# autonomousvision/connecting_the_dots

Measured on AMD Instinct MI355X. Metric: Mpix*disparities/s on 512x432x128 cost volume; disparity MAE vs ref, higher is better.
Workload: dtype f32

## Files before the change

### connecting_the_dots_amd/csrc/argmax_rerank.hip

```cpp
#include "ctd_internal.h"
#include "ctd_ncc_point.h"
#include "ctd_rank.h"
#include "ctd_tail.h"


namespace ctd {

constexpr int kScanBatch = 8;
template <int PX>
__global__ __launch_bounds__(256) __attribute__((amdgpu_waves_per_eu(5, 8))) void argmax_scan_kernel(const float* __restrict__ vol, int64_t* __restrict__ idx,
                                                          float* __restrict__ best, int D, long HW, int W,
                                                          int bs, float eps, long total_threads, WorkList work) {
  const long t = (long)blockIdx.x * blockDim.x + threadIdx.x;
  if (t >= total_threads) return;
  const long p0 = t * PX;
  const long f = p0 / HW, q0 = p0 - f * HW;
  const float* v = vol + f * D * HW + q0;
  const int w0 = (int)(q0 % W);
  float v0[PX], v1[PX];
  int i0[PX], dc[PX];
#pragma unroll
  for (int k = 0; k < PX; ++k) { v0[k] = -INFINITY; v1[k] = -INFINITY; i0[k] = 0; dc[k] = w0 + k + (bs - 1 - bs / 2); }
  constexpr int kBatch = kScanBatch;
  const bool wave_masks = __any(dc[0] < D - 1);
  for (int d0 = 0; d0 < D; d0 += kBatch) {
    float x[kBatch][PX];
#pragma unroll
    for (int u = 0; u < kBatch; ++u) {
      const float* src = v + (long)min(d0 + u, D - 1) * HW;
      if constexpr (PX == 4) {
        typedef float f4 __attribute__((ext_vector_type(4)));
        const f4 q = __builtin_nontemporal_load((const f4*)src);
        x[u][0] = q.x; x[u][1] = q.y; x[u][2] = q.z; x[u][3] = q.w;
      } else if constexpr (PX == 2) {
        typedef float f2 __attribute__((ext_vector_type(2)));
        const f2 q = __builtin_nontemporal_load((const f2*)src);
        x[u][0] = q.x; x[u][1] = q.y;
      } else {
        x[u][0] = __builtin_nontemporal_load(src);
      }
    }
    if (wave_masks || d0 + kBatch > D) {
#pragma unroll
      for (int u = 0; u < kBatch; ++u) {
        const int d = d0 + u;
#pragma unroll
        for (int k = 0; k < PX; ++k) {
          const float y = (d > dc[k] || d >= D) ? -INFINITY : x[u][k];
          v1[k] = __builtin_amdgcn_fmed3f(v0[k], v1[k], y);
          i0[k] = y > v0[k] ? d : i0[k];
          v0[k] = fmaxf(v0[k], y);
        }
      }
    } else {
#pragma unroll
      for (int u = 0; u < kBatch; ++u) {
#pragma unroll
        for (int k = 0; k < PX; ++k) {
          const float y = x[u][k];
          v1[k] = __builtin_amdgcn_fmed3f(v0[k], v1[k], y);
          i0[k] = y > v0[k] ? d0 + u : i0[k];
          v0[k] = fmaxf(v0[k], y);
        }
      }
    }
  }
#pragma unroll
  for (int k = 0; k < PX; ++k) {
    const bool hard = v1[k] >= v0[k] - eps;
    idx[p0 + k] = hard ? (int64_t)(-1 - i0[k]) : (int64_t)i0[k];
    if (best) best[p0 + k] = v0[k];
    if (hard) work.list[atomicAdd(work.counters, 1u)] = p0 + k;
  }
}

constexpr int kMaskWords = 8;

__device__ inline float wave_maxf(float v) {
#pragma unroll
  for (int o = 32; o > 0; o >>= 1) v = fmaxf(v, __shfl_xor(v, o));
  return v;
}

struct RunSource {
  const float* run_vals;
  const float* v1;
  int W1, xoff, per_frame;
};

template <int WORDS, bool VOL>
__device__ __forceinline__ void resolve_role(float* lds_resolve, const float* __restrict__ vol, const float* __restrict__ in0,
                                             const float* __restrict__ in1, long in1_frame_stride,
                                             int64_t* __restrict__ idx, float* __restrict__ best, int D, int H, int W, int bs,
                                             float eps, WorkList work, RunSource rsrc, unsigned role_block,
                                             unsigned n_role_blocks, unsigned waves_used = 4, unsigned* stamp = nullptr) {
  if ((threadIdx.x >> 6) >= waves_used) return;
  const int lane = threadIdx.x & 63;
  const int half = bs / 2, span = bs + D - 1;
  float* sA = lds_resolve + (threadIdx.x >> 6) * 2 * (bs * bs + bs * span);
  float* sB = sA + bs * bs;
  float* sAq = sB + bs * span;
  float* sBq = sAq + bs * bs;
  const float bs2f = (float)(bs * bs);
  const long HW = (long)H * W;
  unsigned seg_cnt[kWorkListParts];
  unsigned longest = 0;
#pragma unroll
  for (int k = 0; k < kWorkListParts; ++k) seg_cnt[k] = work.counters[min(k, work.parts - 1) * kWorkListStride];
#pragma unroll
  for (int k = 0; k < kWorkListParts; ++k) {
    if (k >= work.parts) seg_cnt[k] = 0u;
    longest = max(longest, seg_cnt[k]);
  }
  const unsigned n_slots = longest * (unsigned)work.parts;
  CTD_POST_STAMP_S(stamp, 1, longest);
  const unsigned n_waves = n_role_blocks * waves_used;
  for (unsigned slot = role_block * waves_used + (threadIdx.x >> 6); slot < n_slots; slot += n_waves) {
    const unsigned seg = slot & (unsigned)(work.parts - 1), entry = slot / (unsigned)work.parts;
    unsigned cnt = 0;
#pragma unroll
    for (int k = 0; k < kWorkListParts; ++k) cnt = seg == (unsigned)k ? seg_cnt[k] : cnt;
    if (entry >= cnt) continue;
    const long pj = work.list[(long)seg * work.seg_cap + entry];
    CTD_POST_STAMP_S(stamp, 2, pj);
    CTD_POST_STAMP_ITEM(stamp);
    const long fj = pj / HW, qj = pj - fj * HW;
    const int hj = (int)(qj / W), wj = (int)(qj - (long)hj * W);
    const float* v = VOL ? vol + fj * D * HW + qj : nullptr;
    const int d_clamped = wj + (bs - 1 - bs / 2);
    unsigned long long mask[WORDS];
    int n_cand = 0;
    float x[WORDS];
    bool run_listed = false;
    float rv = 0.f;
    if constexpr (VOL) {
      if (rsrc.run_vals && d_clamped < D) {
        const long z = rsrc.per_frame ? fj : 0;
        run_listed = rsrc.v1[(z * H + hj) * rsrc.W1 + (rsrc.xoff - (bs - 1 - bs / 2))] == 0.f;
        if (run_listed) rv = rsrc.run_vals[(fj * H + hj) * D + d_clamped];
      }
#pragma unroll
      for (int wd = 0; wd < WORDS; ++wd) {
        const int d = min(wd * 64 + lane, D - 1);
        x[wd] = v[(long)(rsrc.run_vals ? min(d, d_clamped) : d) * HW];
        if (run_listed && d >= d_clamped) x[wd] = rv;
      }
      CTD_POST_STAMP_V(stamp, 3, x[0]);
    }
    constexpr int kPreA = 2, kPreB = 20;
    const bool pre = !VOL && bs * bs <= 64 * kPreA && bs * span <= 64 * kPreB;
    const float* a = in0 + fj * HW;
    const float* b = in1 + fj * in1_frame_stride;
    float ta[kPreA], tb[kPreB];
    if (pre) {
#pragma unroll
      for (int k = 0; k < kPreA; ++k) {
        const int i = min(lane + 64 * k, bs * bs - 1);
        const int bh = i / bs, bw = i - bh * bs;
        ta[k] = a[(long)clampi(hj + bh - half, 0, H - 1) * W + clampi(wj + bw - half, 0, W - 1)];
      }
#pragma unroll
      for (int k = 0; k < kPreB; ++k) {
        const int i = min(lane + 64 * k, bs * span - 1);
        const int bh = i / span, c = i - bh * span;
        tb[k] = b[(long)clampi(hj + bh - half, 0, H - 1) * W + clampi(wj - half - (D - 1) + c, 0, W - 1)];
      }
    }
    if constexpr (VOL) {
      float m = -INFINITY;
#pragma unroll
      for (int wd = 0; wd < WORDS; ++wd)
        if (wd * 64 + lane < D && wd * 64 + lane <= d_clamped) m = fmaxf(m, x[wd]);
      m = wave_maxf(m);
      bool have_clamped = false;
#pragma unroll
      for (int wd = 0; wd < WORDS; ++wd) {
        unsigned long long bits = __ballot(wd * 64 + lane < D && x[wd] >= m - eps);
        const int c0 = d_clamped - wd * 64;
        if (c0 < 64) {
          const unsigned long long run = c0 <= 0 ? bits : bits & ~((1ull << c0) - 1ull);
          bits &= ~run;
          if (!have_clamped && run) {
            bits |= run & (0ull - run);
            have_clamped = true;
          }
        }
        mask[wd] = bits;
        n_cand += __popcll(bits);
      }
    } else {
#pragma unroll
      for (int wd = 0; wd < WORDS; ++wd) {
        const int last = min(D - 1, d_clamped) - wd * 64;
        mask[wd] = last < 0 ? 0ull : (last >= 63 ? ~0ull : ((1ull << (last + 1)) - 1ull));
        n_cand += __popcll(mask[wd]);
      }
    }
    float eb = 0.f;
    int ei = 0x7fffffff;
    const bool rescore = VOL ? n_cand > 1 : n_cand >= 1;
    if (rescore && pre) {
#pragma unroll
      for (int k = 0; k < kPreA; ++k)
        if (lane + 64 * k < bs * bs) {
          sA[lane + 64 * k] = ta[k];
          sAq[lane + 64 * k] = ta[k] / bs2f;
        }
#pragma unroll
      for (int k = 0; k < kPreB; ++k)
        if (lane + 64 * k < bs * span) {
          sB[lane + 64 * k] = tb[k];
          sBq[lane + 64 * k] = tb[k] / bs2f;
        }
    } else if (rescore) {
      for (int i = lane; i < bs * bs; i += 64) {
        const int bh = i / bs, bw = i - bh * bs;
        const float xa = a[(long)clampi(hj + bh - half, 0, H - 1) * W + clampi(wj + bw - half, 0, W - 1)];
        sA[i] = xa;
        sAq[i] = xa / bs2f;
      }
      constexpr int NB = 20;
      for (int i0 = lane; i0 < bs * span; i0 += 64 * NB) {
        float t[NB];
#pragma unroll
        for (int k = 0; k < NB; ++k) {
          const int i = min(i0 + 64 * k, bs * span - 1);
          const int bh = i / span, c = i - bh * span;
          t[k] = b[(long)clampi(hj + bh - half, 0, H - 1) * W + clampi(wj - half - (D - 1) + c, 0, W - 1)];
        }
#pragma unroll
        for (int k = 0; k < NB; ++k)
          if (i0 + 64 * k < bs * span) {
            sB[i0 + 64 * k] = t[k];
            sBq[i0 + 64 * k] = t[k] / bs2f;
          }
      }
    }
    CTD_POST_STAMP(stamp, 4);
    if (rescore) {
      for (int c0 = 0; c0 < n_cand; c0 += 64) {
        int my_d = -1, k = 0;
#pragma unroll
        for (int wd = 0; wd < WORDS; ++wd) {
          unsigned long long mj = mask[wd];
          if (k + __popcll(mj) <= c0 || k >= c0 + 64) { k += __popcll(mj); continue; }
          while (mj) {
            const int d = wd * 64 + __ffsll((long long)mj) - 1;
            mj &= mj - 1;
            if (k - c0 == lane) my_d = d;
            ++k;
          }
        }
        float e = -INFINITY;
        if (my_d >= 0) e = bs == 9 ? ncc_exact_point_lds_bs<9>(sA, sB, sAq, sBq, span, (D - 1) - my_d)
                                   : ncc_exact_point_lds(sA, sB, bs, span, (D - 1) - my_d);
        const float em = wave_maxf(e);
        const unsigned long long holders = __ballot(my_d >= 0 && e == em);
        const int dl = __shfl(my_d, holders ? __ffsll((long long)holders) - 1 : 0);
        if (ei == 0x7fffffff || em > eb) { eb = em; ei = dl; }
      }
    } else {
#pragma unroll
      for (int wd = 0; wd < WORDS; ++wd)
        if (mask[wd]) ei = min(ei, wd * 64 + __ffsll((long long)mask[wd]) - 1);
    }
    CTD_POST_STAMP_S(stamp, 5, ei);
    if (lane == 0) {
      idx[pj] = ei;
      if (best) {
        if constexpr (VOL) best[pj] = (run_listed && ei >= d_clamped) ? rv : v[(long)(rsrc.run_vals ? min(ei, d_clamped) : ei) * HW];
        else if (rescore) best[pj] = eb;
      }
    }
    CTD_POST_STAMP(stamp, 6);
    CTD_POST_STAMP(stamp, 9);
    stamp = nullptr;
  }
}

template <int WORDS, bool VOL>
__global__ __launch_bounds__(256) void argmax_resolve_kernel(const float* __restrict__ vol, const float* __restrict__ in0,
                                                             const float* __restrict__ in1, long in1_frame_stride,
                                                             int64_t* __restrict__ idx, float* __restrict__ best, int D,
                                                             int H, int W, int bs, float eps, WorkList work) {
  extern __shared__ float lds_dyn[];
  resolve_role<WORDS, VOL>(lds_dyn, vol, in0, in1, in1_frame_stride, idx, best, D, H, W, bs, eps, work,
                           RunSource{nullptr, nullptr, 0, 0, 0}, blockIdx.x, gridDim.x);
}

constexpr long kResolveBlocks = 1024;
constexpr unsigned kTailResolveWaves = 2;

template <int WORDS, bool VOL>
__global__ __launch_bounds__(256) void rank_tail_kernel(float* __restrict__ vol, const float* __restrict__ in0,
                                                        const float* __restrict__ in1, long in1_frame_stride,
                                                        int64_t* __restrict__ idx, float* __restrict__ best,
                                                        const unsigned char* __restrict__ flags, int frames, int D, int H,
                                                        int W, int bs, float eps, WorkList work, RunSource rsrc,
                                                        unsigned* __restrict__ counters,
                                                        const unsigned long long* __restrict__ run_rows,
                                                        const unsigned long long* __restrict__ flag_a,
                                                        const unsigned long long* __restrict__ flag_b, unsigned n_resolve,
                                                        unsigned n_runs, unsigned n_decode) {
  extern __shared__ float lds_dyn[];
  const unsigned n_pair = min(n_resolve, n_runs);
  unsigned role, rb;
  if (blockIdx.x < n_decode) { role = 2; rb = blockIdx.x; }
  else {
    const unsigned b = blockIdx.x - n_decode;
    if (b < 2 * n_pair) { role = b & 1; rb = b >> 1; }
    else { role = n_resolve > n_runs ? 0 : 1; rb = b - n_pair; }
  }
  if (blockIdx.x == 0 && threadIdx.x == 0) counters[0] = 0u;
  unsigned* stamp = CTD_POST_STAMP_SLOT(role);
  if (role == 0) {
    resolve_role<WORDS, VOL>(lds_dyn, vol, in0, in1, in1_frame_stride, idx, best, D, H, W, bs, eps, work, rsrc, rb, n_resolve,
                             kTailResolveWaves, stamp);
  } else if (role == 1) {
    if constexpr (VOL)
      runs_role(vol, rsrc.run_vals, counters, run_rows, rsrc.per_frame, 1, H, W, D, bs, (int)(rb >> 2), (int)(rb & 3), 4,
                (int*)lds_dyn, stamp);
  } else {
    decode_role((unsigned long long*)idx, best, flags, counters, flag_a, flag_b, rsrc.per_frame, frames, H, W, D,
                rb * 4 + (threadIdx.x >> 6), n_decode * 4, stamp);
  }
}


CTD_POST_STAMP_EXPORT(ctd_debug_read_tail_stamps)

template <bool VOL>
static int launch_resolve(const float* vol, const float* in0, const float* in1, long in1_frame_stride, int64_t* idx,
                          float* best, long total, int D, int H, int W, int bs, float eps, const WorkList& work,
                          hipStream_t stream) {
  const size_t lds = sizeof(float) * 4 * 2 * ((size_t)bs * bs + (size_t)bs * (bs + D - 1));
  if (lds > 160 * 1024) return CTD_ERR_UNSUPPORTED;
  const long chunks = (total + 255) / 256;
  auto resolve = D <= 128 ? argmax_resolve_kernel<2, VOL> : (D <= 256 ? argmax_resolve_kernel<4, VOL> : argmax_resolve_kernel<8, VOL>);
  if (lds > 64 * 1024)
    CTD_HIP_TRY(hipFuncSetAttribute((const void*)resolve, hipFuncAttributeMaxDynamicSharedMemorySize, (int)lds));
  hipLaunchKernelGGL(resolve, dim3((unsigned)(chunks < kResolveBlocks ? chunks : kResolveBlocks)), dim3(256), lds, stream, vol,
                     in0, in1, in1_frame_stride, idx, best, D, H, W, bs, eps, work);
  CTD_LAUNCH_CHECK();
  return CTD_OK;
}

template <bool VOL>
static int launch_tail(const RankPlan& rp, float* vol, const float* in0, const float* in1, long in1_frame_stride,
                       int64_t* idx, float* best, int frames, int D, int H, int W, int bs, hipStream_t stream) {
  size_t lds = sizeof(float) * kTailResolveWaves * 2 * ((size_t)bs * bs + (size_t)bs * (bs + D - 1));
  if (lds < sizeof(int) * (size_t)H) lds = sizeof(int) * (size_t)H;
  if (lds > 160 * 1024) return CTD_ERR_UNSUPPORTED;
  const long total = (long)frames * H * W;
  const long chunks = (total + 255) / 256;
  const unsigned n_resolve = rp.eps >= 0.f ? (unsigned)(chunks < kResolveBlocks ? chunks : kResolveBlocks) : 0u;
  const unsigned n_runs = VOL ? (unsigned)(frames * ceil_div(D, kRunPlanes)) * 4u : 0u;
  const unsigned n_decode = 128u;
  auto kern = D <= 128 ? rank_tail_kernel<2, VOL> : (D <= 256 ? rank_tail_kernel<4, VOL> : rank_tail_kernel<8, VOL>);
  if (lds > 64 * 1024)
    CTD_HIP_TRY(hipFuncSetAttribute((const void*)kern, hipFuncAttributeMaxDynamicSharedMemorySize, (int)lds));
  const RunSource rsrc = {rp.run_vals, rp.v1, rp.W1, rp.xoff, in1_frame_stride != 0 ? 1 : 0};
  hipLaunchKernelGGL(kern, dim3(n_resolve + n_runs + n_decode), dim3(256), lds, stream, vol, in0, in1, in1_frame_stride, idx,
                     best, rp.flags, frames, D, H, W, bs, rp.eps, rp.work, rsrc, rp.counters, rp.run_rows, rp.flag_a, rp.flag_b,
                     n_resolve,
                     n_runs, n_decode);
  CTD_LAUNCH_CHECK();
  return CTD_OK;
}

int rank_tail_f32(const RankPlan& rp, float* vol, const float* in0, const float* in1, long in1_frame_stride, int64_t* idx,
                  float* best, int frames, int D, int H, int W, int bs, hipStream_t stream) {
  return vol ? launch_tail<true>(rp, vol, in0, in1, in1_frame_stride, idx, best, frames, D, H, W, bs, stream)
             : launch_tail<false>(rp, nullptr, in0, in1, in1_frame_stride, idx, best, frames, D, H, W, bs, stream);
}

int argmax_rerank_f32(const float* vol, const float* in0, const float* in1, long in1_frame_stride, int64_t* idx,
                      float* best, int frames, int D, int H, int W, int bs, float eps, void* workspace,
                      size_t workspace_bytes, bool counter_cleared, hipStream_t stream) {
  if (D > kMaskWords * 64) return CTD_ERR_UNSUPPORTED;
  const long total = (long)frames * H * W;
  const long HW = (long)H * W;
  if (!workspace || workspace_bytes < 16 + sizeof(int64_t) * (size_t)total) return CTD_ERR_WORKSPACE;
  unsigned* n_hard = (unsigned*)workspace;
  const WorkList work = {n_hard, (int64_t*)((char*)workspace + 16), 1, W, total};
  if (!counter_cleared) CTD_HIP_TRY(hipMemsetAsync(n_hard, 0, 16, stream));
  const bool vec4 = W % 4 == 0 && ((uintptr_t)vol % 16) == 0;
  const int px = vec4 ? 4 : 1;
  if (px == 4)
    hipLaunchKernelGGL(argmax_scan_kernel<4>, dim3((unsigned)((total / 4 + 255) / 256)), dim3(256), 0, stream, vol,
                       idx, best, D, HW, W, bs, eps, total / 4, work);
  else
    hipLaunchKernelGGL(argmax_scan_kernel<1>, dim3((unsigned)((total + 255) / 256)), dim3(256), 0, stream, vol, idx,
                       best, D, HW, W, bs, eps, total, work);
  CTD_LAUNCH_CHECK();
  if (eps < 0.f) return CTD_OK;
  return launch_resolve<true>(vol, in0, in1, in1_frame_stride, idx, best, total, D, H, W, bs, eps, work, stream);
}

}
```

### connecting_the_dots_amd/csrc/ctd_ncc_point.h

```cpp
#ifndef CTD_NCC_POINT_H
#define CTD_NCC_POINT_H
#include "ctd_common.h"

namespace ctd {

__device__ inline float ncc_norm(float s0, float s1) {
  return (float)((double)sqrtf(s0 * s1) + 1e-8);
}
__device__ inline double ncc_norm(double s0, double s1) { return sqrt(s0 * s1) + 1e-8; }

__device__ inline float ncc_exact_term_lds(const float* sA, const float* sB, int bs, int span, int off) {
  const float bs2 = (float)(bs * bs);
  float mu0 = 0.f, mu1 = 0.f;
  for (int bh = 0; bh < bs; ++bh)
    for (int bw = 0; bw < bs; ++bw) {
      mu0 += sA[bh * bs + bw] / bs2;
      mu1 += sB[bh * span + bw + off] / bs2;
    }
  float s0 = 0.f, s1 = 0.f, dot = 0.f;
  for (int bh = 0; bh < bs; ++bh)
    for (int bw = 0; bw < bs; ++bw) {
      const float v0 = sA[bh * bs + bw] - mu0;
      const float v1 = sB[bh * span + bw + off] - mu1;
      dot += v0 * v1;
      s0 += v0 * v0;
      s1 += v1 * v1;
    }
  return dot / ncc_norm(s0, s1);
}
__device__ inline float ncc_exact_point_lds(const float* sA, const float* sB, int bs, int span, int off) {
  float val = 0.f;
  val += ncc_exact_term_lds(sA, sB, bs, span, off);
  return val;
}

template <int BS>
__device__ inline float ncc_exact_point_lds_bs(const float* sA, const float* sB, const float* sAq, const float* sBq,
                                               int span, int off) {
  float mu0 = 0.f, mu1 = 0.f;
  for (int bh = 0; bh < BS; ++bh) {
    float a[BS], b[BS];
#pragma unroll
    for (int bw = 0; bw < BS; ++bw) { a[bw] = sAq[bh * BS + bw]; b[bw] = sBq[bh * span + bw + off]; }
#pragma unroll
    for (int bw = 0; bw < BS; ++bw) {
      mu0 += a[bw];
      mu1 += b[bw];
    }
  }
  float s0 = 0.f, s1 = 0.f, dot = 0.f;
  for (int bh = 0; bh < BS; ++bh) {
    float a[BS], b[BS];
#pragma unroll
    for (int bw = 0; bw < BS; ++bw) { a[bw] = sA[bh * BS + bw]; b[bw] = sB[bh * span + bw + off]; }
#pragma unroll
    for (int bw = 0; bw < BS; ++bw) {
      const float v0 = a[bw] - mu0;
      const float v1 = b[bw] - mu1;
      dot += v0 * v1;
      s0 += v0 * v0;
      s1 += v1 * v1;
    }
  }
  float val = 0.f;
  val += dot / ncc_norm(s0, s1);
  return val;
}

}
#endif
```

Measured before the change: 1.001 million.

## Halve resolve LDS footprint, restage quotient buffers, and size tail grid by occupancy

The resolve role now keeps a single pair of LDS tile buffers per wave. For bs=9 it first fills them with pre-divided values to compute the means, then reloads the raw values to compute the centred NCC, instead of holding separate quotient copies. This halves the tail kernel's LDS and lets all four waves per block resolve where only two did before. The change also adds a waves-per-EU hint, readfirstlane and bpermute/readlane wave primitives, and row-relative 32-bit addressing. Run-role sharing now shrinks so the whole grid fits the occupancy the device admits, at the cost of reloading the B tile from global memory a second time.

```diff
diff --git a/connecting_the_dots_amd/csrc/argmax_rerank.hip b/connecting_the_dots_amd/csrc/argmax_rerank.hip
--- a/connecting_the_dots_amd/csrc/argmax_rerank.hip
+++ b/connecting_the_dots_amd/csrc/argmax_rerank.hip
@@ -76,10 +76,17 @@
 
 constexpr int kMaskWords = 8;
 
-__device__ inline float wave_maxf(float v) {
-#pragma unroll
-  for (int o = 32; o > 0; o >>= 1) v = fmaxf(v, __shfl_xor(v, o));
+__device__ inline float wave_maxf(float v, int lane) {
+#pragma unroll
+  for (int o = 32; o > 0; o >>= 1)
+    v = fmaxf(v, __int_as_float(__builtin_amdgcn_ds_bpermute((lane ^ o) << 2, __float_as_int(v))));
   return v;
+}
+
+__device__ __forceinline__ unsigned wave_uniform(unsigned v) { return (unsigned)__builtin_amdgcn_readfirstlane((int)v); }
+__device__ __forceinline__ long wave_uniform(long v) {
+  const unsigned lo = wave_uniform((unsigned)v), hi = wave_uniform((unsigned)((unsigned long long)v >> 32));
+  return (long)(((unsigned long long)hi << 32) | lo);
 }
 
 struct RunSource {
@@ -88,19 +95,54 @@
   int W1, xoff, per_frame;
 };
 
+__device__ __forceinline__ unsigned resolve_a_offset(int i, int hj, int wj, int bs, int half, int H, int W, int r0) {
+  const int bh = i / bs, bw = i - bh * bs;
+  return (unsigned)((clampi(hj + bh - half, 0, H - 1) - r0) * W + clampi(wj + bw - half, 0, W - 1));
+}
+__device__ __forceinline__ unsigned resolve_b_offset(int i, int hj, int wj, int span, int half, int D, int H, int W, int r0) {
+  const int bh = i / span, c = i - bh * span;
+  return (unsigned)((clampi(hj + bh - half, 0, H - 1) - r0) * W + clampi(wj - half - (D - 1) + c, 0, W - 1));
+}
+template <int N>
+__device__ __forceinline__ void resolve_load_batch(float (&t)[N], const float* __restrict__ img, int ln, int cols, int hj,
+                                                   int col0, int bs, int half, int H, int W, int r0) {
+  const int qs = 64 / cols, rs = 64 - qs * cols;
+  int r = ln / cols, c = ln - r * cols;
+#pragma unroll
+  for (int k = 0; k < N; ++k) {
+    t[k] = img[(unsigned)((clampi(hj + min(r, bs - 1) - half, 0, H - 1) - r0) * W + clampi(col0 + c, 0, W - 1))];
+    c += rs;
+    r += qs;
+    if (c >= cols) { c -= cols; ++r; }
+  }
+}
+
+template <int FIRST, int N, class Offset>
+__device__ __forceinline__ void resolve_stage_rest(float* s, const float* __restrict__ img, int lane, int n, bool quot,
+                                                   float bs2f, Offset offset) {
+  for (int base = 64 * FIRST; base < n; base += 64 * N) {
+    float t[N];
+#pragma unroll
+    for (int k = 0; k < N; ++k) t[k] = img[offset(min(base + lane + 64 * k, n - 1))];
+#pragma unroll
+    for (int k = 0; k < N; ++k)
+      if (base + lane + 64 * k < n) s[base + lane + 64 * k] = quot ? t[k] / bs2f : t[k];
+  }
+}
+
 template <int WORDS, bool VOL>
 __device__ __forceinline__ void resolve_role(float* lds_resolve, const float* __restrict__ vol, const float* __restrict__ in0,
                                              const float* __restrict__ in1, long in1_frame_stride,
                                              int64_t* __restrict__ idx, float* __restrict__ best, int D, int H, int W, int bs,
                                              float eps, WorkList work, RunSource rsrc, unsigned role_block,
-                                             unsigned n_role_blocks, unsigned waves_used = 4, unsigned* stamp = nullptr) {
-  if ((threadIdx.x >> 6) >= waves_used) return;
+                                             unsigned n_role_blocks, unsigned* stamp = nullptr) {
   const int lane = threadIdx.x & 63;
+  const unsigned wave = (unsigned)__builtin_amdgcn_readfirstlane((int)(threadIdx.x >> 6));
   const int half = bs / 2, span = bs + D - 1;
-  float* sA = lds_resolve + (threadIdx.x >> 6) * 2 * (bs * bs + bs * span);
-  float* sB = sA + bs * bs;
-  float* sAq = sB + bs * span;
-  float* sBq = sAq + bs * bs;
+  const int n_a = bs * bs, n_b = bs * span;
+  float* sA = lds_resolve + wave * (n_a + n_b);
+  float* sB = sA + n_a;
+  const bool quot = bs == 9;
   const float bs2f = (float)(bs * bs);
   const long HW = (long)H * W;
   unsigned seg_cnt[kWorkListParts];
@@ -108,20 +150,17 @@
 #pragma unroll
   for (int k = 0; k < kWorkListParts; ++k) seg_cnt[k] = work.counters[min(k, work.parts - 1) * kWorkListStride];
 #pragma unroll
-  for (int k = 0; k < kWorkListParts; ++k) {
-    if (k >= work.parts) seg_cnt[k] = 0u;
-    longest = max(longest, seg_cnt[k]);
-  }
-  const unsigned n_slots = longest * (unsigned)work.parts;
+  for (int k = 0; k < kWorkListParts; ++k) longest = max(longest, k < work.parts ? seg_cnt[k] : 0u);
+  const unsigned n_slots = wave_uniform(longest) * (unsigned)work.parts;
   CTD_POST_STAMP_S(stamp, 1, longest);
-  const unsigned n_waves = n_role_blocks * waves_used;
-  for (unsigned slot = role_block * waves_used + (threadIdx.x >> 6); slot < n_slots; slot += n_waves) {
+  const unsigned n_waves = n_role_blocks * 4u;
+  for (unsigned slot = role_block * 4u + wave; slot < n_slots; slot += n_waves) {
     const unsigned seg = slot & (unsigned)(work.parts - 1), entry = slot / (unsigned)work.parts;
-    unsigned cnt = 0;
-#pragma unroll
-    for (int k = 0; k < kWorkListParts; ++k) cnt = seg == (unsigned)k ? seg_cnt[k] : cnt;
+    const unsigned cnt = wave_uniform(work.counters[seg * kWorkListStride]);
+    const long pj = wave_uniform(work.list[(long)seg * work.seg_cap + entry]);
     if (entry >= cnt) continue;
-    const long pj = work.list[(long)seg * work.seg_cap + entry];
+    int ln = lane;
+    asm volatile("" : "+v"(ln));
     CTD_POST_STAMP_S(stamp, 2, pj);
     CTD_POST_STAMP_ITEM(stamp);
     const long fj = pj / HW, qj = pj - fj * HW;
@@ -141,41 +180,25 @@
       }
 #pragma unroll
       for (int wd = 0; wd < WORDS; ++wd) {
-        const int d = min(wd * 64 + lane, D - 1);
+        const int d = min(wd * 64 + ln, D - 1);
         x[wd] = v[(long)(rsrc.run_vals ? min(d, d_clamped) : d) * HW];
         if (run_listed && d >= d_clamped) x[wd] = rv;
       }
       CTD_POST_STAMP_V(stamp, 3, x[0]);
     }
-    constexpr int kPreA = 2, kPreB = 20;
-    const bool pre = !VOL && bs * bs <= 64 * kPreA && bs * span <= 64 * kPreB;
-    const float* a = in0 + fj * HW;
-    const float* b = in1 + fj * in1_frame_stride;
-    float ta[kPreA], tb[kPreB];
-    if (pre) {
-#pragma unroll
-      for (int k = 0; k < kPreA; ++k) {
-        const int i = min(lane + 64 * k, bs * bs - 1);
-        const int bh = i / bs, bw = i - bh * bs;
-        ta[k] = a[(long)clampi(hj + bh - half, 0, H - 1) * W + clampi(wj + bw - half, 0, W - 1)];
-      }
-#pragma unroll
-      for (int k = 0; k < kPreB; ++k) {
-        const int i = min(lane + 64 * k, bs * span - 1);
-        const int bh = i / span, c = i - bh * span;
-        tb[k] = b[(long)clampi(hj + bh - half, 0, H - 1) * W + clampi(wj - half - (D - 1) + c, 0, W - 1)];
-      }
-    }
+    const int r0 = clampi(hj - half, 0, H - 1);
+    const float* a = in0 + fj * HW + (long)r0 * W;
+    const float* b = in1 + fj * in1_frame_stride + (long)r0 * W;
     if constexpr (VOL) {
       float m = -INFINITY;
 #pragma unroll
       for (int wd = 0; wd < WORDS; ++wd)
-        if (wd * 64 + lane < D && wd * 64 + lane <= d_clamped) m = fmaxf(m, x[wd]);
-      m = wave_maxf(m);
+        if (wd * 64 + ln < D && wd * 64 + ln <= d_clamped) m = fmaxf(m, x[wd]);
+      m = wave_maxf(m, ln);
       bool have_clamped = false;
 #pragma unroll
       for (int wd = 0; wd < WORDS; ++wd) {
-        unsigned long long bits = __ballot(wd * 64 + lane < D && x[wd] >= m - eps);
+        unsigned long long bits = __ballot(wd * 64 + ln < D && x[wd] >= m - eps);
         const int c0 = d_clamped - wd * 64;
         if (c0 < 64) {
           const unsigned long long run = c0 <= 0 ? bits : bits & ~((1ull << c0) - 1ull);
@@ -199,46 +222,27 @@
     float eb = 0.f;
     int ei = 0x7fffffff;
     const bool rescore = VOL ? n_cand > 1 : n_cand >= 1;
-    if (rescore && pre) {
-#pragma unroll
-      for (int k = 0; k < kPreA; ++k)
-        if (lane + 64 * k < bs * bs) {
-          sA[lane + 64 * k] = ta[k];
-          sAq[lane + 64 * k] = ta[k] / bs2f;
-        }
-#pragma unroll
-      for (int k = 0; k < kPreB; ++k)
-        if (lane + 64 * k < bs * span) {
-          sB[lane + 64 * k] = tb[k];
-          sBq[lane + 64 * k] = tb[k] / bs2f;
-        }
-    } else if (rescore) {
-      for (int i = lane; i < bs * bs; i += 64) {
-        const int bh = i / bs, bw = i - bh * bs;
-        const float xa = a[(long)clampi(hj + bh - half, 0, H - 1) * W + clampi(wj + bw - half, 0, W - 1)];
-        sA[i] = xa;
-        sAq[i] = xa / bs2f;
-      }
-      constexpr int NB = 20;
-      for (int i0 = lane; i0 < bs * span; i0 += 64 * NB) {
-        float t[NB];
-#pragma unroll
-        for (int k = 0; k < NB; ++k) {
-          const int i = min(i0 + 64 * k, bs * span - 1);
-          const int bh = i / span, c = i - bh * span;
-          t[k] = b[(long)clampi(hj + bh - half, 0, H - 1) * W + clampi(wj - half - (D - 1) + c, 0, W - 1)];
-        }
-#pragma unroll
-        for (int k = 0; k < NB; ++k)
-          if (i0 + 64 * k < bs * span) {
-            sB[i0 + 64 * k] = t[k];
-            sBq[i0 + 64 * k] = t[k] / bs2f;
-          }
-      }
+    constexpr int NA = 2, NB = 20, NR = WORDS == 2 ? 4 : NB;
+    float ta[NA], tb[NB];
+    if (rescore) {
+      resolve_load_batch(ta, a, ln, bs, hj, wj - half, bs, half, H, W, r0);
+      resolve_load_batch(tb, b, ln, span, hj, wj - half - (D - 1), bs, half, H, W, r0);
+#pragma unroll
+      for (int k = 0; k < NA; ++k)
+        if (ln + 64 * k < n_a) sA[ln + 64 * k] = quot ? ta[k] / bs2f : ta[k];
+#pragma unroll
+      for (int k = 0; k < NB; ++k)
+        if (ln + 64 * k < n_b) sB[ln + 64 * k] = quot ? tb[k] / bs2f : tb[k];
+      resolve_stage_rest<NA, NA>(sA, a, ln, n_a, quot, bs2f, [&](int i) { return resolve_a_offset(i, hj, wj, bs, half, H, W, r0); });
+      resolve_stage_rest<NB, NR>(sB, b, ln, n_b, quot, bs2f, [&](int i) { return resolve_b_offset(i, hj, wj, span, half, D, H, W, r0); });
     }
     CTD_POST_STAMP(stamp, 4);
     if (rescore) {
-      for (int c0 = 0; c0 < n_cand; c0 += 64) {
+      int my_ds[WORDS];
+      float mu1s[WORDS], mu0 = 0.f;
+#pragma unroll
+      for (int r = 0; r < WORDS; ++r) { my_ds[r] = -1; mu1s[r] = 0.f; }
+      for (int c0 = 0, r = 0; c0 < n_cand; c0 += 64, ++r) {
         int my_d = -1, k = 0;
 #pragma unroll
         for (int wd = 0; wd < WORDS; ++wd) {
@@ -247,16 +251,38 @@
           while (mj) {
             const int d = wd * 64 + __ffsll((long long)mj) - 1;
             mj &= mj - 1;
-            if (k - c0 == lane) my_d = d;
+            if (k - c0 == ln) my_d = d;
             ++k;
           }
         }
+        float m0 = 0.f, m1 = 0.f;
+        if (quot && my_d >= 0) ncc_exact_means_lds_bs<9>(sA, sB, span, (D - 1) - my_d, m0, m1);
+        if (r == 0) mu0 = m0;
+#pragma unroll
+        for (int q = 0; q < WORDS; ++q)
+          if (q == r) { my_ds[q] = my_d; mu1s[q] = m1; }
+      }
+      if (quot) {
+#pragma unroll
+        for (int k = 0; k < NA; ++k)
+          if (ln + 64 * k < n_a) sA[ln + 64 * k] = ta[k];
+#pragma unroll
+        for (int k = 0; k < NB; ++k)
+          if (ln + 64 * k < n_b) sB[ln + 64 * k] = tb[k];
+        resolve_stage_rest<NB, NR>(sB, b, ln, n_b, false, bs2f, [&](int i) { return resolve_b_offset(i, hj, wj, span, half, D, H, W, r0); });
+      }
+      for (int c0 = 0, r = 0; c0 < n_cand; c0 += 64, ++r) {
+        int my_d = -1;
+        float mu1 = 0.f;
+#pragma unroll
+        for (int q = 0; q < WORDS; ++q)
+          if (q == r) { my_d = my_ds[q]; mu1 = mu1s[q]; }
         float e = -INFINITY;
-        if (my_d >= 0) e = bs == 9 ? ncc_exact_point_lds_bs<9>(sA, sB, sAq, sBq, span, (D - 1) - my_d)
-                                   : ncc_exact_point_lds(sA, sB, bs, span, (D - 1) - my_d);
-        const float em = wave_maxf(e);
+        if (my_d >= 0) e = quot ? ncc_exact_centred_lds_bs<9>(sA, sB, span, (D - 1) - my_d, mu0, mu1)
+                                : ncc_exact_point_lds(sA, sB, bs, span, (D - 1) - my_d);
+        const float em = wave_maxf(e, ln);
         const unsigned long long holders = __ballot(my_d >= 0 && e == em);
-        const int dl = __shfl(my_d, holders ? __ffsll((long long)holders) - 1 : 0);
+        const int dl = __builtin_amdgcn_readlane(my_d, holders ? __ffsll((long long)holders) - 1 : 0);
         if (ei == 0x7fffffff || em > eb) { eb = em; ei = dl; }
       }
     } else {
@@ -265,7 +291,7 @@
         if (mask[wd]) ei = min(ei, wd * 64 + __ffsll((long long)mask[wd]) - 1);
     }
     CTD_POST_STAMP_S(stamp, 5, ei);
-    if (lane == 0) {
+    if (ln == 0) {
       idx[pj] = ei;
       if (best) {
         if constexpr (VOL) best[pj] = (run_listed && ei >= d_clamped) ? rv : v[(long)(rsrc.run_vals ? min(ei, d_clamped) : ei) * HW];
@@ -289,19 +315,19 @@
 }
 
 constexpr long kResolveBlocks = 1024;
-constexpr unsigned kTailResolveWaves = 2;
+constexpr long kTailResolveBlocks = kResolveBlocks / 2;
+
+__host__ __device__ constexpr int tail_waves_per_simd(int words) { return words == 2 ? 7 : 5; }
 
 template <int WORDS, bool VOL>
-__global__ __launch_bounds__(256) void rank_tail_kernel(float* __restrict__ vol, const float* __restrict__ in0,
-                                                        const float* __restrict__ in1, long in1_frame_stride,
-                                                        int64_t* __restrict__ idx, float* __restrict__ best,
-                                                        const unsigned char* __restrict__ flags, int frames, int D, int H,
-                                                        int W, int bs, float eps, WorkList work, RunSource rsrc,
-                                                        unsigned* __restrict__ counters,
-                                                        const unsigned long long* __restrict__ run_rows,
-                                                        const unsigned long long* __restrict__ flag_a,
-                                                        const unsigned long long* __restrict__ flag_b, unsigned n_resolve,
-                                                        unsigned n_runs, unsigned n_decode) {
+__global__ __launch_bounds__(256) __attribute__((amdgpu_waves_per_eu(tail_waves_per_simd(WORDS))))
+void rank_tail_kernel(float* __restrict__ vol, const float* __restrict__ in0, const float* __restrict__ in1,
+                      long in1_frame_stride, int64_t* __restrict__ idx, float* __restrict__ best,
+                      const unsigned char* __restrict__ flags, int frames, int D, int H, int W, int bs, float eps,
+                      WorkList work, RunSource rsrc, unsigned* __restrict__ counters,
+                      const unsigned long long* __restrict__ run_rows, const unsigned long long* __restrict__ flag_a,
+                      const unsigned long long* __restrict__ flag_b, unsigned n_resolve, unsigned n_runs,
+                      unsigned n_decode, unsigned run_shares) {
   extern __shared__ float lds_dyn[];
   const unsigned n_pair = min(n_resolve, n_runs);
   unsigned role, rb;
@@ -315,11 +341,11 @@
   unsigned* stamp = CTD_POST_STAMP_SLOT(role);
   if (role == 0) {
     resolve_role<WORDS, VOL>(lds_dyn, vol, in0, in1, in1_frame_stride, idx, best, D, H, W, bs, eps, work, rsrc, rb, n_resolve,
-                             kTailResolveWaves, stamp);
+                             stamp);
   } else if (role == 1) {
     if constexpr (VOL)
-      runs_role(vol, rsrc.run_vals, counters, run_rows, rsrc.per_frame, 1, H, W, D, bs, (int)(rb >> 2), (int)(rb & 3), 4,
-                (int*)lds_dyn, stamp);
+      runs_role(vol, rsrc.run_vals, counters, run_rows, rsrc.per_frame, 1, H, W, D, bs, (int)(rb / run_shares),
+                (int)(rb % run_shares), (int)run_shares, (int*)lds_dyn, stamp);
   } else {
     decode_role((unsigned long long*)idx, best, flags, counters, flag_a, flag_b, rsrc.per_frame, frames, H, W, D,
                 rb * 4 + (threadIdx.x >> 6), n_decode * 4, stamp);
@@ -333,7 +359,7 @@
 static int launch_resolve(const float* vol, const float* in0, const float* in1, long in1_frame_stride, int64_t* idx,
                           float* best, long total, int D, int H, int W, int bs, float eps, const WorkList& work,
                           hipStream_t stream) {
-  const size_t lds = sizeof(float) * 4 * 2 * ((size_t)bs * bs + (size_t)bs * (bs + D - 1));
+  const size_t lds = sizeof(float) * 4 * ((size_t)bs * bs + (size_t)bs * (bs + D - 1));
   if (lds > 160 * 1024) return CTD_ERR_UNSUPPORTED;
   const long chunks = (total + 255) / 256;
   auto resolve = D <= 128 ? argmax_resolve_kernel<2, VOL> : (D <= 256 ? argmax_resolve_kernel<4, VOL> : argmax_resolve_kernel<8, VOL>);
@@ -348,22 +374,27 @@
 template <bool VOL>
 static int launch_tail(const RankPlan& rp, float* vol, const float* in0, const float* in1, long in1_frame_stride,
                        int64_t* idx, float* best, int frames, int D, int H, int W, int bs, hipStream_t stream) {
-  size_t lds = sizeof(float) * kTailResolveWaves * 2 * ((size_t)bs * bs + (size_t)bs * (bs + D - 1));
+  size_t lds = sizeof(float) * 4 * ((size_t)bs * bs + (size_t)bs * (bs + D - 1));
   if (lds < sizeof(int) * (size_t)H) lds = sizeof(int) * (size_t)H;
   if (lds > 160 * 1024) return CTD_ERR_UNSUPPORTED;
   const long total = (long)frames * H * W;
   const long chunks = (total + 255) / 256;
-  const unsigned n_resolve = rp.eps >= 0.f ? (unsigned)(chunks < kResolveBlocks ? chunks : kResolveBlocks) : 0u;
-  const unsigned n_runs = VOL ? (unsigned)(frames * ceil_div(D, kRunPlanes)) * 4u : 0u;
+  const unsigned n_resolve = rp.eps >= 0.f ? (unsigned)(chunks < kTailResolveBlocks ? chunks : kTailResolveBlocks) : 0u;
   const unsigned n_decode = 128u;
+  const int words = D <= 128 ? 2 : (D <= 256 ? 4 : 8);
+  const long by_lds = (long)(160 * 1024 / lds), by_regs = tail_waves_per_simd(words);
+  const long admitted = (by_lds < by_regs ? by_lds : by_regs) * device_cu_count();
+  const unsigned run_groups = VOL ? (unsigned)(frames * ceil_div(D, kRunPlanes)) : 0u;
+  unsigned run_shares = 4u;
+  while (run_shares > 1u && (long)n_resolve + (long)run_groups * run_shares + n_decode > admitted) run_shares >>= 1;
+  const unsigned n_runs = run_groups * run_shares;
   auto kern = D <= 128 ? rank_tail_kernel<2, VOL> : (D <= 256 ? rank_tail_kernel<4, VOL> : rank_tail_kernel<8, VOL>);
   if (lds > 64 * 1024)
     CTD_HIP_TRY(hipFuncSetAttribute((const void*)kern, hipFuncAttributeMaxDynamicSharedMemorySize, (int)lds));
   const RunSource rsrc = {rp.run_vals, rp.v1, rp.W1, rp.xoff, in1_frame_stride != 0 ? 1 : 0};
   hipLaunchKernelGGL(kern, dim3(n_resolve + n_runs + n_decode), dim3(256), lds, stream, vol, in0, in1, in1_frame_stride, idx,
                      best, rp.flags, frames, D, H, W, bs, rp.eps, rp.work, rsrc, rp.counters, rp.run_rows, rp.flag_a, rp.flag_b,
-                     n_resolve,
-                     n_runs, n_decode);
+                     n_resolve, n_runs, n_decode, run_shares);
   CTD_LAUNCH_CHECK();
   return CTD_OK;
 }
diff --git a/connecting_the_dots_amd/csrc/ctd_ncc_point.h b/connecting_the_dots_amd/csrc/ctd_ncc_point.h
--- a/connecting_the_dots_amd/csrc/ctd_ncc_point.h
+++ b/connecting_the_dots_amd/csrc/ctd_ncc_point.h
@@ -35,8 +35,8 @@
 }
 
 template <int BS>
-__device__ inline float ncc_exact_point_lds_bs(const float* sA, const float* sB, const float* sAq, const float* sBq,
-                                               int span, int off) {
+__device__ inline void ncc_exact_means_lds_bs(const float* sAq, const float* sBq, int span, int off, float& mu0_out,
+                                              float& mu1_out) {
   float mu0 = 0.f, mu1 = 0.f;
   for (int bh = 0; bh < BS; ++bh) {
     float a[BS], b[BS];
@@ -48,6 +48,12 @@
       mu1 += b[bw];
     }
   }
+  mu0_out = mu0;
+  mu1_out = mu1;
+}
+
+template <int BS>
+__device__ inline float ncc_exact_centred_lds_bs(const float* sA, const float* sB, int span, int off, float mu0, float mu1) {
   float s0 = 0.f, s1 = 0.f, dot = 0.f;
   for (int bh = 0; bh < BS; ++bh) {
     float a[BS], b[BS];
```

Result: no change. 997,500 (-0.3%).
